# grossjohannes/AlignNet-3D

Hardware: AMD Instinct MI355X
Metric: point-cloud pairs/sec at N=1024 (inference, eval-mode forward) (higher is better)
Workload: dtype f32; 1 GPU; SynthCars widths inference, batch=256 pairs/GPU, N=1024, fp32 (BASELINE.json configs[1]); pairs_per_gpu=256, num_points=1024, parallelism=batch-split x1 (no collective)

## Files before the change

### alignnet-3d_amd/csrc/alignnet_api.hip

```cpp
#include "engine.h"
#include "kernels_infer.h"
#include "kernels_dgcnn.h"
#include "kernels_infer_split.h"
#include "kernels_dgcnn_split.h"

#include <algorithm>
#include <cmath>
#include <cstdio>
#include <cstring>
#include <random>

using namespace alignnet;

static thread_local std::string g_create_err;

#define HIP_TRY(h, expr)                                                                         \
  do {                                                                                           \
    hipError_t e_ = (expr);                                                                      \
    if (e_ != hipSuccess) {                                                                      \
      (h)->err = std::string(#expr) + ": " + hipGetErrorString(e_);                              \
      return 1;                                                                                  \
    }                                                                                            \
  } while (0)

// ... 343 lines not shown
    const size_t o_xform = tot; tot += al(B2 * 12);
    const size_t o_cm = tot; tot += al(B2 * 3);
    const size_t o_s1c = tot; tot += al(B2 * 3);
    const size_t o_s2c = tot; tot += al(B2 * 3);
    const size_t o_theta = tot; tot += al(B2);
    const size_t o_cls = tot; tot += al(B2);
    const size_t o_p1 = tot; tot += al(B2 * C1);
    const size_t o_p2 = tot; tot += al(B2 * C2);
    const size_t o_emb = tot; tot += al(B2 * CE);
    const size_t o_hs = tot; tot += al(B2 * H);
    const size_t o_ha = tot; tot += al(B2 * H);
    const size_t o_hb = tot; tot += al(B2 * H);
    const size_t o_o1 = tot; tot += al(B2 * 3);
    const size_t o_o2 = tot; tot += al(B2 * (3 + nb2));
    const size_t o_o3 = tot; tot += al((size_t)B * (3 + nb2));
    size_t o_out[8];
    const int widths[8] = {3, nb2, 3, 3, 3, 3, nb2, nb2};
    for (int i = 0; i < 8; ++i) { o_out[i] = tot; tot += al((size_t)B * widths[i]); }
    if (!(o_hs >= o_p1 && o_hs + al(B2 * H) <= o_ha)) return fail(h, "workspace carve: hid_s must lie inside the range the centroid kernel clears ([pool1, hid_a))");
    HIP_TRY(h, hipMalloc(&w.d_all, tot * sizeof(float)));
    float* base = w.d_all;
    w.xform = base + o_xform; w.center_mean = base + o_cm; w.s1c = base + o_s1c; w.s2c = base + o_s2c;
    w.theta = base + o_theta; w.cls = reinterpret_cast<int*>(base + o_cls);
    w.pool1 = base + o_p1; w.pool2 = base + o_p2; w.emb = base + o_emb;
    w.hid_a = base + o_ha; w.hid_b = base + o_hb; w.hid_s = base + o_hs;
    w.o1 = base + o_o1; w.o2 = base + o_o2; w.o3 = base + o_o3;
    for (int i = 0; i < 8; ++i) w.outs[i] = base + o_out[i];
    w.cap = B;
  }
  if (h->cfg.backbone == 1 && !w.d_nn) {
    HIP_TRY(h, hipMalloc(&w.d_nn, (size_t)2 * w.cap * N * 20 * sizeof(int)));
  }
  if (need_inputs && !w.d_pcs[0]) {
    for (int t = 0; t < 2; ++t) HIP_TRY(h, hipMalloc(&w.d_pcs[t], (size_t)w.cap * N * 3 * sizeof(float)));
  }
  return 0;
}

static int infer_tile_pts(const alignnet_handle* h, int B)
{
  if (h->ab & AB_INFER_TILE64) return 64;
  if (h->infer_tile_opt) return h->infer_tile_opt;
  const long tiles128 = (long)2 * B * ((h->cfg.num_points + 127) / 128);
  return tiles128 <= 128 ? 64 : 128;
}

static size_t backbone_lds_bytes(const alignnet_handle* h, const Stack& st, int ld[2], int B)
{
  const int kTilePts = infer_tile_pts(h, B);
  int w[2] = {8, 8};
  for (int i = 0; i < st.n - 1; ++i) w[i & 1] = std::max(w[i & 1], (h->layers[st.first + i].cout + 7) & ~7);
  ld[0] = w[0] + 4; ld[1] = w[1] + 4;
  return ((size_t)kTilePts * 4 + (size_t)kTilePts * (ld[0] + ld[1])) * sizeof(float);
}

static int run_backbone(alignnet_handle* h, const Stack& st, const float* p1, const float* p2, int B, float* pooled,
                        long tower_stride, long row_stride, size_t pooled_floats)
{
  BackboneArgs a;
  a.pcs[0] = p1; a.pcs[1] = p2; a.xform = h->ws.xform; a.pooled = pooled;
  a.tower_stride = tower_stride; a.row_stride = row_stride;
  a.B = B; a.N = h->cfg.num_points; a.nlayers = st.n;
  const size_t lds = backbone_lds_bytes(h, st, a.ld, B);
  if (lds > 160 * 1024) return fail(h, "backbone hidden widths need more than 160 KiB of LDS per 128-point tile");
  for (int i = 0; i < st.n; ++i) {
    const Layer& L = h->layers[st.first + i];
    a.L[i].w = L.first_conv ? h->d_params + h->params[L.p_w].offset : h->d_wp + L.off_wp;
    a.L[i].scale = h->d_scale + L.off_ss;
    a.L[i].shift = h->d_shift + L.off_ss;
    a.L[i].cin = L.cin; a.L[i].cout = L.cout;
  }
  (void)pooled_floats;
#ifdef ALIGNNET_KSTAMP
  static long long* d_stamps = nullptr;
  if (!d_stamps) { hipMalloc(&d_stamps, 4 * 64 * sizeof(long long)); }
  hipMemsetAsync(d_stamps, 0, 4 * 64 * sizeof(long long), h->stream);
  a.stamps = d_stamps;
#endif
  static PerDeviceOnce attr_set;
  if (attr_set.need(h->cfg.device)) {
    HIP_TRY(h, hipFuncSetAttribute(reinterpret_cast<const void*>(pointnet_fused<128>), hipFuncAttributeMaxDynamicSharedMemorySize, 160 * 1024));
    HIP_TRY(h, hipFuncSetAttribute(reinterpret_cast<const void*>(pointnet_fused<128, 68, 132>), hipFuncAttributeMaxDynamicSharedMemorySize, 160 * 1024));
    HIP_TRY(h, hipFuncSetAttribute(reinterpret_cast<const void*>(pointnet_fused<128, 68, 132, 16>), hipFuncAttributeMaxDynamicSharedMemorySize, 160 * 1024));
    HIP_TRY(h, hipFuncSetAttribute(reinterpret_cast<const void*>(pointnet_fused<64>), hipFuncAttributeMaxDynamicSharedMemorySize, 160 * 1024));
    HIP_TRY(h, hipFuncSetAttribute(reinterpret_cast<const void*>(pointnet_fused<64, 68, 132, 16>), hipFuncAttributeMaxDynamicSharedMemorySize, 160 * 1024));
    attr_set.mark(h->cfg.device);
  }
  const int TP = infer_tile_pts(h, B);
  const int ntiles = (a.N + TP - 1) / TP;
  int per = ntiles;
  while (per > 1 && (long)2 * B * ((ntiles + per - 1) / per) < 512) per = (per + 1) / 2;
  if (h->ab_tiles_per_wg > 0) per = std::min(ntiles, h->ab_tiles_per_wg);
  a.tiles_per_wg = per;
  const dim3 grid((ntiles + per - 1) / per, 2 * B);
  {
  ProfScope prof_scope(h, PK_BACKBONE, true);
  const int sc1 = h->layers[st.first].cout, sc2 = st.n == 3 ? h->layers[st.first + 1].cout : 0;
  if (h->infer_split && st.n == 3 && sc1 <= 16 * kSplitKB1 && sc2 <= 16 * kSplitKB2) {
    SplitArgs sa;
    sa.pcs[0] = p1; sa.pcs[1] = p2; sa.xform = a.xform; sa.pooled = pooled; sa.tower_stride = tower_stride; sa.row_stride = row_stride;
    sa.B = B; sa.N = a.N; sa.C1 = sc1; sa.C2 = sc2; sa.C3 = h->layers[st.first + 2].cout;
    sa.w1 = a.L[0].w; sa.w2s = h->d_wps + h->off_wps[st.first + 1]; sa.w3s = h->d_wps + h->off_wps[st.first + 2];
    sa.dbg = h->ablate_dbg & 0xff;
    if (h->ablate_dbg >> 8) sa.prio_mask = (h->ablate_dbg >> 8) & 0xff;
    sa.sc1 = a.L[0].scale; sa.sh1 = a.L[0].shift; sa.sc2 = a.L[1].scale; sa.sh2 = a.L[1].shift; sa.sc3 = a.L[2].scale; sa.sh3 = a.L[2].shift;
    const int ld1s = ((sc1 + 15) & ~15) + 8, ld2s = ((sc2 + 15) & ~15) + 8;
    const size_t slds = (size_t)kSplitTP * 4 * sizeof(float) + (size_t)2 * kSplitTP * (ld1s + ld2s) * sizeof(unsigned short);
    static PerDeviceOnce sattr;
    if (sattr.need(h->cfg.device)) { HIP_TRY(h, hipFuncSetAttribute(reinterpret_cast<const void*>(pointnet_split<>), hipFuncAttributeMaxDynamicSharedMemorySize, 160 * 1024)); sattr.mark(h->cfg.device); }
    if (sc1 == 64 && sc2 == 128 && sa.C3 % 64 == 0 && sa.C3 >= 256 && split_persist_lds(sa.C3).total_bytes <= 160 * 1024 && !(h->ab & (AB_NO_LD_CONST | AB_SPLIT_TILEWISE))) {
      static PerDeviceOnce pattr;
      static int cus[64];
      if (pattr.need(h->cfg.device)) {
        HIP_TRY(h, hipFuncSetAttribute(reinterpret_cast<const void*>(pointnet_split_persist<4>), hipFuncAttributeMaxDynamicSharedMemorySize, 160 * 1024));
        HIP_TRY(h, hipFuncSetAttribute(reinterpret_cast<const void*>(pointnet_split_persist<2>), hipFuncAttributeMaxDynamicSharedMemorySize, 160 * 1024));
        int n = 0;
        HIP_TRY(h, hipDeviceGetAttribute(&n, hipDeviceAttributeMultiprocessorCount, h->cfg.device));
        cus[h->cfg.device & 63] = n > 0 ? n : 256;
        pattr.mark(h->cfg.device);
      }
      const long tiles = (long)2 * B * ((a.N + kSplitTP - 1) / kSplitTP);
      const int wgs = (int)std::min<long>(tiles, cus[h->cfg.device & 63]);
      {
#ifdef ALIGNNET_ABLATE
      if ((sa.dbg & 64) && sa.C3 == 1024) { sa.stamps = reinterpret_cast<long long*>(h->ws.hid_a); hipMemsetAsync(sa.stamps, 0, 8 * 16 * sizeof(long long), h->stream); }
#endif
      if (sa.C3 >= 512) { TIMED_LAUNCH(pointnet_split_persist<4>, dim3(wgs), dim3(kWaves * 64), (size_t)split_persist_lds(sa.C3).total_bytes, sa); }
      else { TIMED_LAUNCH(pointnet_split_persist<2>, dim3(wgs), dim3(kWaves * 64), (size_t)split_persist_lds(sa.C3).total_bytes, sa); }
      h->last_kernel = ALIGNNET_KERNEL_POINTNET_SPLIT_PERSIST;
#ifdef ALIGNNET_ABLATE
      if (sa.stamps) {
        long long hs[8 * 16];
        hipStreamSynchronize(h->stream);
        hipMemcpy(hs, sa.stamps, sizeof(hs), hipMemcpyDeviceToHost);
        for (int w = 0; w < 8; ++w) {
          std::fprintf(stderr, "psp wave %d: start +%lld |", w, hs[w * 16] - hs[0]);
          for (int i = 1; i < 7; ++i) std::fprintf(stderr, " %lld", hs[w * 16 + i] - hs[w * 16 + i - 1]);
          std::fprintf(stderr, "   (xs+barrier, lift, barrier, hidden, barrier, last layer)\n");
        }
      }
#endif
      }
    } else if (sc1 == 64 && sc2 == 128 && !(h->ab & AB_NO_LD_CONST)) {
      static PerDeviceOnce sattr;
      if (sattr.need(h->cfg.device)) { HIP_TRY(h, hipFuncSetAttribute(reinterpret_cast<const void*>(pointnet_split<64, 128>), hipFuncAttributeMaxDynamicSharedMemorySize, 160 * 1024)); sattr.mark(h->cfg.device); }
      TIMED_LAUNCH((pointnet_split<64, 128>), dim3((a.N + kSplitTP - 1) / kSplitTP, 2 * B), dim3(kWaves * 64), slds, sa);
      h->last_kernel = ALIGNNET_KERNEL_POINTNET_SPLIT_64_128;
    } else {
      TIMED_LAUNCH(pointnet_split<>, dim3((a.N + kSplitTP - 1) / kSplitTP, 2 * B), dim3(kWaves * 64), slds, sa);
      h->last_kernel = ALIGNNET_KERNEL_POINTNET_SPLIT;
    }
  } else if (TP == 64 && !(h->ab & AB_INFER_TILE64) && a.ld[0] == 68 && a.ld[1] == 132 && st.n == 3 && h->layers[st.first + 2].cin == 128 && !(h->ab & AB_NO_LD_CONST)) {
    TIMED_LAUNCH((pointnet_fused<64, 68, 132, 16>), grid, dim3(kWaves * 64), lds, a);
    h->last_kernel = ALIGNNET_KERNEL_POINTNET_FUSED_64_128_K16_TP64;
  } else if (TP == 64) { TIMED_LAUNCH(pointnet_fused<64>, grid, dim3(kWaves * 64), lds, a); h->last_kernel = ALIGNNET_KERNEL_POINTNET_FUSED_TP64; }
  else if (a.ld[0] == 68 && a.ld[1] == 132 && st.n == 3 && h->layers[st.first + 2].cin == 128 && !(h->ab & AB_NO_LD_CONST)) {
    TIMED_LAUNCH((pointnet_fused<128, 68, 132, 16>), grid, dim3(kWaves * 64), lds, a);
    h->last_kernel = ALIGNNET_KERNEL_POINTNET_FUSED_64_128_K16;
  } else if (a.ld[0] == 68 && a.ld[1] == 132 && !(h->ab & AB_NO_LD_CONST)) {
    TIMED_LAUNCH((pointnet_fused<128, 68, 132>), grid, dim3(kWaves * 64), lds, a);
    h->last_kernel = ALIGNNET_KERNEL_POINTNET_FUSED_64_128;
  } else { TIMED_LAUNCH(pointnet_fused<128>, grid, dim3(kWaves * 64), lds, a); h->last_kernel = ALIGNNET_KERNEL_POINTNET_FUSED; }
  }
  HIP_TRY(h, hipGetLastError());
#ifdef ALIGNNET_KSTAMP
  if (st.first == h->emb_conv.first && true) {
    long long hs[4 * 64];
    hipStreamSynchronize(h->stream);
    hipMemcpy(hs, d_stamps, sizeof(hs), hipMemcpyDeviceToHost);
    for (int q = 0; q < 4; ++q) {
      std::fprintf(stderr, "wave %d ct %d:", (q >> 1) * 4, (q & 1) * 8 + (q >> 1) * 4);
      for (int i = 1; i < 64 && hs[q * 64 + i]; ++i) std::fprintf(stderr, " %lld", hs[q * 64 + i] - hs[q * 64 + i - 1]);
      std::fprintf(stderr, "  | first %lld\n", hs[q * 64] - hs[0]);
    }
  }
#endif
  return 0;
}

static int run_backbone_dgcnn(alignnet_handle* h, const Stack& st, const float* p1, const float* p2, int B, float* pooled,
                              long tower_stride, long row_stride, size_t pooled_floats)
{
  DgcnnArgs a;
  a.stamps = nullptr;
  a.pcs[0] = p1; a.pcs[1] = p2; a.xform = h->ws.xform; a.nn = h->ws.d_nn; a.pooled = pooled;
  a.tower_stride = tower_stride; a.row_stride = row_stride;
  a.B = B; a.N = h->cfg.num_points; a.k = 20; a.nlayers = st.n;
  int wmax[2] = {8, 8};
  for (int i = 0; i < st.n - 1; ++i) wmax[i & 1] = std::max(wmax[i & 1], (h->layers[st.first + i].cout + 7) & ~7);
  a.ld[0] = wmax[0] + 4; a.ld[1] = wmax[1] + 4;
  const bool dg_std = a.ld[0] == 68 && a.ld[1] == 132 && st.n == 3 && !(h->ab & AB_NO_LD_CONST);
  const size_t lds = dg_std ? ((size_t)kDgTile * 9 + (size_t)kDgTile * 68 + 4 * 8 * 64 * 4) * sizeof(float)
                            : ((size_t)kDgTile * 16 + (size_t)kDgTile * (2 * a.ld[0] + a.ld[1])) * sizeof(float);
  if (lds > 160 * 1024) return fail(h, "dgcnn hidden widths need more than 160 KiB of LDS per 64-point tile");
  if (h->layers[st.first + st.n - 2].cout > 256) return fail(h, "dgcnn: last edge-conv width limited to 256 channels");
  for (int i = 0; i < st.n; ++i) {
    const Layer& L = h->layers[st.first + i];
    a.L[i].w = L.first_conv ? h->d_params + h->params[L.p_w].offset : h->d_wp + L.off_wp;
    a.L[i].scale = h->d_scale + L.off_ss;
    a.L[i].shift = h->d_shift + L.off_ss;
    a.L[i].cin = L.cin; a.L[i].cout = L.cout;
  }
  (void)pooled_floats;
  static PerDeviceOnce attr_set;
  if (attr_set.need(h->cfg.device)) {
    HIP_TRY(h, hipFuncSetAttribute(reinterpret_cast<const void*>(dgcnn_fused<>), hipFuncAttributeMaxDynamicSharedMemorySize, 160 * 1024));
    attr_set.mark(h->cfg.device);
  }
  const dim3 grid((a.N + kDgTile - 1) / kDgTile, 2 * B);
  {
  ProfScope prof_scope(h, PK_BACKBONE, true);
  {
    const int dca = h->layers[st.first].cout, dcb = st.n == 3 ? h->layers[st.first + 1].cout : 0;
    if (h->infer_split && st.n == 3 && dca <= 16 * kSplitKB1 && dcb <= 128) {
      DgcnnSplitArgs sa;
      sa.pcs[0] = p1; sa.pcs[1] = p2; sa.xform = a.xform; sa.nn = a.nn; sa.pooled = pooled; sa.tower_stride = tower_stride; sa.row_stride = row_stride;
      sa.B = B; sa.N = a.N; sa.k = a.k; sa.Ca = dca; sa.Cb = dcb; sa.C3 = h->layers[st.first + 2].cout;
      sa.w1 = a.L[0].w; sa.w2s = h->d_wps + h->off_wps[st.first + 1]; sa.w3s = h->d_wps + h->off_wps[st.first + 2];
      sa.sc1 = a.L[0].scale; sa.sh1 = a.L[0].shift; sa.sc2 = a.L[1].scale; sa.sh2 = a.L[1].shift; sa.sc3 = a.L[2].scale; sa.sh3 = a.L[2].shift;
      sa.dbg = h->ablate_dbg;
      const int dlda = ((dca + 15) & ~15) + 8, dldb = ((dcb + 15) & ~15) + 8;
      if (a.k > 3 * kWaves) return fail(h, "dgcnn split kernel: k limited to 24 neighbours");
      const size_t dlds = (size_t)2 * kDgTile * 8 * sizeof(float) + ((size_t)4 * kDgTile * dlda + (size_t)2 * kDgTile * dldb) * sizeof(unsigned short);
      static PerDeviceOnce dsattr;
      if (dsattr.need(h->cfg.device)) { HIP_TRY(h, hipFuncSetAttribute(reinterpret_cast<const void*>(dgcnn_split<>), hipFuncAttributeMaxDynamicSharedMemorySize, 160 * 1024)); dsattr.mark(h->cfg.device); }
      if (dca == 64 && dcb == 128 && !(h->ab & AB_NO_LD_CONST)) {
        static PerDeviceOnce dsattr2;
        if (dsattr2.need(h->cfg.device)) { HIP_TRY(h, hipFuncSetAttribute(reinterpret_cast<const void*>(dgcnn_split<64, 128>), hipFuncAttributeMaxDynamicSharedMemorySize, 160 * 1024)); dsattr2.mark(h->cfg.device); }
        TIMED_LAUNCH((dgcnn_split<64, 128>), grid, dim3(kWaves * 64), dlds, sa);
        h->last_kernel = ALIGNNET_KERNEL_DGCNN_SPLIT_64_128;
      } else {
        TIMED_LAUNCH(dgcnn_split<>, grid, dim3(kWaves * 64), dlds, sa);
        h->last_kernel = ALIGNNET_KERNEL_DGCNN_SPLIT;
      }
    } else {
      const int dbg = h->ablate_dbg;
      a.stamps = (dbg & 64) ? reinterpret_cast<long long*>(h->ws.hid_a) : nullptr;
      if (a.ld[0] == 68 && a.ld[1] == 132 && st.n == 3 && !(h->ab & AB_NO_LD_CONST)) {
        static PerDeviceOnce sattr;
        if (sattr.need(h->cfg.device)) { HIP_TRY(h, hipFuncSetAttribute(reinterpret_cast<const void*>(dgcnn_fused<68, 132>), hipFuncAttributeMaxDynamicSharedMemorySize, 160 * 1024)); sattr.mark(h->cfg.device); }
// ... 455 lines not shown
```

### alignnet-3d_amd/csrc/engine.h

```cpp
#pragma once
#include <hip/hip_runtime.h>
#include <hip/hip_ext.h>
#include <stdint.h>
#include <string>
#include <vector>
#include <map>
#include <atomic>

#include "../../include/alignnet_hip.h"

namespace alignnet {

struct ParamInfo {
  std::string name;
  int rows, cols;
  bool trainable;
  size_t offset;
  size_t count() const { return (size_t)rows * cols; }
};

struct Layer {
  std::string name;
  int cin, cout;
  bool bn, siamese, conv, first_conv;
  int fan_in, fan_out;
  int p_w, p_b;
  int p_bn[2][4];
  size_t off_wp;
  size_t off_ss;
};

struct Stack { int first, n; };

enum ProfKernel { PK_BACKBONE = 0, PK_KNN, PK_TRAIN_PHASE2, PK_TRAIN_PHASE3, PK_TRAIN_GRAM, PK_TRAIN_B2, PK_TRAIN_B1, PK_DG_FWD, PK_DG_BWD_EDGE,
                  PK_ALLREDUCE, PK_OPTIMIZER, PK_SCENE_WINDOW, PK_SCENE_CAST, PK_SCENE_COMPACT, PK_ICP_GRID_BUILD, PK_ICP_GRID, PK_SCENE_BIN, PK_ICP_PLANE_NORMALS, PK_ICP_PLANE, PK_SCENE_BAND, PK_TRACKLET_TEST, PK_TRACKLET_COMPACT, PK_COUNT };
static const char* const kProfKernelNames[PK_COUNT] = {"backbone", "knn", "train_fwd_phase2", "train_fwd_phase3", "train_gram_h2", "train_bwd_b2",
                                                       "train_bwd_b1", "dg_train_fwd", "dg_train_bwd_edge", "allreduce", "optimizer", "scene_window", "scene_cast", "scene_compact", "icp_grid_build", "icp_grid", "scene_bin", "icp_plane_normals", "icp_plane", "scene_band", "tracklet_test", "tracklet_compact"};

constexpr int kTrackletChunk = 1024;
constexpr int kTrackletJobsPerPass = 32;

struct Workspace {
  int cap = 0;
  float* d_pcs[2] = {nullptr, nullptr};
  int* d_nn = nullptr;
  float* d_all = nullptr;
  float *xform, *center_mean, *s1c, *s2c, *theta;
  int* cls;
  float *pool1, *pool2, *emb;
  float *hid_a, *hid_b;
  float* hid_s;
  bool hid_s_zeroed = false;
  float *o1, *o2, *o3;
  float* outs[8];
};

}

namespace alignnet {
struct DatasetTables { const float* pts[2]; const long long* off; long long n; const long long* h_off; const float* labels; };
struct SampleSource { const float* pts[2]; const long long* off; const float* labels; const int* rows; const long long* streams; };
struct IcpDeviceIo {
  const double* init; double* out; double* fitness; double* rmse; int* iters;
  long long* ws_off;
  std::vector<long long>* h_ws_off;
};
}
enum AbBit : unsigned {
  AB_NO_LD_CONST = 1u << 0,
  AB_INFER_TILE64 = 1u << 1,
  AB_PHASE2_LEGACY = 1u << 2,
  AB_B1_LEGACY = 1u << 3,
  AB_B1_FP32 = 1u << 4,
  AB_P3BF16_GENERIC = 1u << 5,
  AB_P3_NOGRAM = 1u << 6,
  AB_NO_DEFER = 1u << 7,
  AB_DG_SPARSE = 1u << 8,
  AB_NO_GLUE_FOLD = 1u << 9,
  AB_FC_DIRECT = 1u << 11,
  AB_FC_NO_SPLITK = 1u << 12,
  AB_SPLIT_TILEWISE = 1u << 13,
  AB_GEMM_JOBS_KSPLIT = 1u << 10,
};
static const struct { const char* key; unsigned bit; } kAbKeys[] = {
  {"ab_no_ld_const", AB_NO_LD_CONST}, {"ab_infer_tile64", AB_INFER_TILE64}, {"ab_phase2_legacy", AB_PHASE2_LEGACY}, {"ab_b1_legacy", AB_B1_LEGACY},
  {"ab_b1_fp32", AB_B1_FP32}, {"ab_p3_bf16_generic", AB_P3BF16_GENERIC}, {"ab_p3_nogram", AB_P3_NOGRAM}, {"ab_no_defer", AB_NO_DEFER},
  {"ab_dg_sparse", AB_DG_SPARSE}, {"ab_no_glue_fold", AB_NO_GLUE_FOLD}, {"ab_gemm_jobs_ksplit", AB_GEMM_JOBS_KSPLIT}, {"ab_fc_direct", AB_FC_DIRECT}, {"ab_fc_no_splitk", AB_FC_NO_SPLITK}, {"ab_split_tilewise", AB_SPLIT_TILEWISE}};
struct alignnet_handle;
bool alignnet_dataset_tables(alignnet_handle* h, alignnet::DatasetTables* out);
int alignnet_dataset_install(alignnet_handle* h, const float* points1, const float* points2, bool device_points, const int64_t* offsets, const float* labels,
                             int64_t n_examples, const char* fn);
int alignnet_dataset_sample_launch(alignnet_handle* h, const alignnet::SampleSource& s, int B, int cap, uint64_t seed, float* out0, float* out1,
                                   float* lab, alignnet_labels* lab_ptrs);
int alignnet_icp_run_device(alignnet_handle* h, const float* const pts[2], const long long* off, const int* rows, const long long* n2, long long stage_n2,
                            int B, const alignnet::IcpDeviceIo& io, double radius, double normal_radius, int its, bool full, bool plane);
size_t alignnet_eval_loss_work_floats(int B);
int alignnet_eval_loss_launch(alignnet_handle* h, const alignnet_labels* d_labels, int B, float* d_work);
void alignnet_register_free(alignnet_handle* h);
int alignnet_drain_profile(alignnet_handle* h);
int alignnet_train_set_option(alignnet_handle* h, const std::string& key, int64_t value);
int alignnet_train_get_option(alignnet_handle* h, const std::string& key, int64_t* value);

struct alignnet_handle {
  alignnet_config cfg;
  std::vector<alignnet::Layer> layers;
  alignnet::Stack s1_conv, s1_fc, s2_conv, s2_fc, emb_conv, rem_fc;
  std::vector<alignnet::ParamInfo> params;
  std::map<std::string, int> by_name;
  size_t n_trainable = 0, n_total = 0;
  float* d_params = nullptr;
  float* d_wp = nullptr;
  float* d_scale = nullptr;
  float* d_shift = nullptr;
  size_t n_wp = 0, n_ss = 0;
  bool infer_split = false;
  unsigned short* d_wps = nullptr;
  std::vector<size_t> off_wps;
  bool train_bf16 = false;
  bool fused_tail = true;
  bool train_ws_stale = false;
  bool folded = false;
  alignnet::Workspace ws;
  hipStream_t stream = nullptr;
  int64_t step = 0;
  uint64_t dropout_stream = 0;
  float adam_b1p = 1.f, adam_b2p = 1.f;
  int64_t adam_power_t = 0;
  int last_B = 0;
  int last_kernel = 0;
  int last_train_B = 0;
  int last_train_kernel = 0;
  bool prof = false;
  hipEvent_t ev[2] = {nullptr, nullptr};
  double prof_backbone_ms = 0, prof_total_ms = 0;
  int64_t prof_backbone_launches = 0;
  struct ProfEv { int id; hipEvent_t a, b; };
  std::vector<ProfEv> prof_pending;
  std::vector<std::pair<hipEvent_t, hipEvent_t>> prof_pool;
  double prof_ms[alignnet::PK_COUNT] = {0};
  int64_t prof_launches[alignnet::PK_COUNT] = {0};
  void* train_ws = nullptr;
  void* dataset_ws = nullptr;
  void* globalreg_ws = nullptr;
  size_t globalreg_ws_bytes = 0;
  int icp_search = 0;
  void* register_ws = nullptr;
  void* icp_grid_ws = nullptr;
  size_t icp_grid_ws_bytes = 0, icp_grid_ws_used = 0;
  size_t icp_plane_ws_budget = 0;
  int icp_plane_chunks = 0;
  int scene_cast = 0;
  int scene_rows = 0;
  int scene_binned_clouds = 0;
  long long scene_bin_entries = 0;
  void* scene_ws = nullptr;
  void* tracklet_ws = nullptr;
  void* pipe = nullptr;
  uint64_t dropout_seed_base() const { return (cfg.seed + dropout_stream * 0xD1B54A32D192ED03ull) * 0x9E3779B97F4A7C15ull + (uint64_t)step * 16; }
  void* comm = nullptr;
  void* comm_grad = nullptr;
  int comm_world = 1, comm_rank = 0;
  hipStream_t comm_stream = nullptr;
  hipEvent_t comm_ev[4] = {nullptr, nullptr, nullptr, nullptr};
  bool comm_overlap = true;
  hipStream_t side_stream = nullptr;
  hipEvent_t side_ev[4] = {nullptr, nullptr, nullptr, nullptr};
  int dw_side = 0;
  unsigned ab = 0;
  int infer_tile_opt = 0;
  int dg_parts_opt = 0;
// ... 45 lines not shown
```

### alignnet-3d_amd/csrc/kernels_infer.h

```cpp
#pragma once
#include <hip/hip_runtime.h>
#include <stdint.h>

namespace alignnet {

typedef __attribute__((ext_vector_type(16))) float f32x16;
typedef __attribute__((ext_vector_type(4))) float f32x4;

constexpr int kTilePts = 128;
constexpr int kWaves = 8;
constexpr int kMaxConv = 6;
constexpr float kBnEps = 1e-3f;

#ifndef ALIGNNET_NO_SETPRIO
#define ALIGNNET_SETPRIO 1
#endif

[[maybe_unused]] static __global__ void pack_weights_kernel(const float* __restrict__ W, int K, int C, float* __restrict__ Wp)
{
  const int KG = (K + 7) >> 3, CT = (C + 31) >> 5;
  const size_t total = (size_t)CT * KG * 256;
  for (size_t idx = blockIdx.x * (size_t)blockDim.x + threadIdx.x; idx < total; idx += (size_t)gridDim.x * blockDim.x) {
    const int s = idx & 3, lane = (idx >> 2) & 63;
    const size_t t = idx >> 8;
// ... 181 lines not shown
    b2 = wload_issue(wp + min(kg + 2, last) * 64);
    lds_rows<MR>(arow, lda, min(kg + 1, last), a1);
    wload_wait2(b0);
    KSTAMP();
    mfma_kgroup<MR>(a0, b0, acc);
    KSTAMP();
    b0 = wload_issue(wp + min(kg + 3, last) * 64);
    lds_rows<MR>(arow, lda, min(kg + 2, last), a0);
    wload_wait2(b1);
    if (kg + 1 < KG) mfma_kgroup<MR>(a1, b1, acc);
    b1 = wload_issue(wp + min(kg + 4, last) * 64);
    lds_rows<MR>(arow, lda, min(kg + 3, last), a1);
    wload_wait2(b2);
    if (kg + 2 < KG) mfma_kgroup<MR>(a0, b2, acc);
#pragma unroll
    for (int m = 0; m < MR; ++m) a0[m] = a1[m];
  }
  KSTAMP();
  wload_drain(b0, b1, b2);
  KSTAMP();
}

template <int MR, bool CLEAR = true>
__device__ __forceinline__ void mfma_rows_deep(const float* __restrict__ A, int lda, const f32x4* __restrict__ Wp, int KG, int lane,
                                               f32x16 (&acc)[MR])
{
  if (CLEAR) {
#pragma unroll
    for (int m = 0; m < MR; ++m)
#pragma unroll
      for (int r = 0; r < 16; ++r) acc[m][r] = 0.f;
  }
  const float* arow = A + (lane & 31) * lda + (lane >> 5) * 4;
  const f32x4* wp = Wp + lane;
  const int last = KG - 1;
  f32x4 b0 = wp[0], b1 = wp[min(1, last) * 64], b2 = wp[min(2, last) * 64];
  asm volatile("" ::: "memory");
  f32x4 av[MR];
  for (int kg = 0; kg < KG; kg += 3) {
    lds_rows<MR>(arow, lda, kg, av);
    mfma_kgroup<MR>(av, b0, acc);
    b0 = wp[min(kg + 3, last) * 64];
    asm volatile("" ::: "memory");
    if (kg + 1 < KG) { lds_rows<MR>(arow, lda, kg + 1, av); mfma_kgroup<MR>(av, b1, acc); }
    b1 = wp[min(kg + 4, last) * 64];
    asm volatile("" ::: "memory");
    if (kg + 2 < KG) { lds_rows<MR>(arow, lda, kg + 2, av); mfma_kgroup<MR>(av, b2, acc); }
    b2 = wp[min(kg + 5, last) * 64];
    asm volatile("" ::: "memory");
  }
}

template <int MR, int KGC = 0>
__device__ __forceinline__ void hidden_item(const float* __restrict__ in, int ldi, float* __restrict__ out, int ldo,
                                            const ConvLayerDev& L, int tower, int ct, int rg, int lane)
{
  const int KG = KGC ? KGC : (L.cin + 7) >> 3;
  f32x16 acc[MR];
  mfma_rows<MR>(in + rg * MR * 32 * ldi, ldi, reinterpret_cast<const f32x4*>(L.w) + (size_t)ct * KG * 64, KG, lane, acc);
  const int col = ct * 32 + (lane & 31);
  const bool live = col < L.cout;
  const float sc = live ? L.scale[tower * L.cout + col] : 0.f;
  const float sh = live ? L.shift[tower * L.cout + col] : 0.f;
  if (col < ldo - 4) {
#pragma unroll
    for (int m = 0; m < MR; ++m)
#pragma unroll
      for (int r = 0; r < 16; ++r) {
        const int row = (rg * MR + m) * 32 + (r & 3) + 8 * (r >> 2) + 4 * (lane >> 5);
        out[row * ldo + col] = fmaxf(fmaf(acc[m][r], sc, sh), 0.f);
      }
  }
}

template <int MR, int TP>
__device__ __forceinline__ void hidden_layer(const float* in, int ldi, float* out, int ldo, const ConvLayerDev& L,
                                             int tower, int wave, int lane)
{
  constexpr int RG = (TP / 32) / MR;
  const int CT = (L.cout + 31) >> 5;
  for (int item = wave; item < CT * RG; item += kWaves) hidden_item<MR>(in, ldi, out, ldo, L, tower, item / RG, item % RG, lane);
}

template <int TP, int LD0 = 0, int LD1 = 0, int KGL = 0>
__global__ __launch_bounds__(kWaves * 64, 2) void pointnet_fused(const BackboneArgs a)
{
  const int lds_ld[2] = {LD0 ? LD0 : a.ld[0], LD1 ? LD1 : a.ld[1]};
  extern __shared__ __attribute__((aligned(16))) float smem[];
  const int tid = threadIdx.x, lane = tid & 63;
  const int wave = __builtin_amdgcn_readfirstlane(tid >> 6);
  const int cloud = blockIdx.y;
  const int tower = cloud >= a.B, b = cloud - tower * a.B;
  float* xs = smem;
  const int boff[2] = {TP * 4, TP * 4 + TP * lds_ld[0]};
  constexpr int kPoolRegs = 4;
  float pool[kPoolRegs] = {0.f, 0.f, 0.f, 0.f};
  const int ntiles_all = (a.N + TP - 1) / TP;
  const int tile_lo = blockIdx.x * a.tiles_per_wg, tile_hi = min(ntiles_all, tile_lo + a.tiles_per_wg);
  float nx = 0.f, ny = 0.f, nz = 0.f;
  auto request_xyz = [&](int t) {
    if (tid < TP) {
      const int n = min(t * TP + tid, a.N - 1);
      const float* p = a.pcs[tower] + ((size_t)b * a.N + n) * 3;
      nx = p[0]; ny = p[1]; nz = p[2];
    }
  };
  request_xyz(tile_lo);
  float l0w[2][5];
#pragma unroll
  for (int g = 0; g < 2; ++g) {
    const ConvLayerDev& L0 = a.L[0];
    const int c = (tid & 31) + 32 * g;
    const bool live = c < L0.cout;
    l0w[g][0] = live ? L0.w[c] : 0.f; l0w[g][1] = live ? L0.w[L0.cout + c] : 0.f; l0w[g][2] = live ? L0.w[2 * L0.cout + c] : 0.f;
    l0w[g][3] = live ? L0.scale[tower * L0.cout + c] : 0.f; l0w[g][4] = live ? L0.shift[tower * L0.cout + c] : 0.f;
  }
  for (int tile = tile_lo; tile < tile_hi; ++tile) {
  if (tile != tile_lo) __syncthreads();

  if (tid < TP) {
    const float* xf = a.xform + (size_t)cloud * 12;
    const float x = nx - xf[0], y = ny - xf[1], z = nz - xf[2];
    xs[tid * 4 + 0] = x * xf[3] + y * xf[6] + z * xf[9];
    xs[tid * 4 + 1] = x * xf[4] + y * xf[7] + z * xf[10];
    xs[tid * 4 + 2] = x * xf[5] + y * xf[8] + z * xf[11];
  }
  if (tile + 1 < tile_hi) request_xyz(tile + 1);
  __syncthreads();

  {
    const ConvLayerDev& L = a.L[0];
    float* out = smem + boff[0];
    const int ldo = lds_ld[0], c0 = tid & 31, r0 = tid >> 5;
    for (int c = c0; c < ldo - 4; c += 32) {
      const bool live = c < L.cout;
      const int g = (c - c0) >> 5;
      float w0, w1, w2, sc, sh;
      if (g < 2) { w0 = g ? l0w[1][0] : l0w[0][0]; w1 = g ? l0w[1][1] : l0w[0][1]; w2 = g ? l0w[1][2] : l0w[0][2];
                   sc = g ? l0w[1][3] : l0w[0][3]; sh = g ? l0w[1][4] : l0w[0][4]; }
      else { w0 = live ? L.w[c] : 0.f; w1 = live ? L.w[L.cout + c] : 0.f; w2 = live ? L.w[2 * L.cout + c] : 0.f;
             sc = live ? L.scale[tower * L.cout + c] : 0.f; sh = live ? L.shift[tower * L.cout + c] : 0.f; }
#pragma unroll
      for (int rr = 0; rr < TP / 16; ++rr) {
        const int row = rr * 16 + r0;
        const f32x4 p = *reinterpret_cast<const f32x4*>(xs + row * 4);
        const float acc = fmaf(p[2], w2, fmaf(p[1], w1, p[0] * w0));
        out[row * ldo + c] = fmaxf(fmaf(acc, sc, sh), 0.f);
      }
    }
  }
  __syncthreads();

  if constexpr (KGL != 0 && LD0 != 0 && LD1 != 0) {
    constexpr int CTH = (LD1 - 4) / 32, RGH = (TP / 32) / 2;
    for (int item = wave; item < CTH * RGH; item += kWaves)
      hidden_item<2, (LD0 - 4) / 8>(smem + boff[0], LD0, smem + boff[1], LD1, a.L[1], tower, item / RGH, item % RGH, lane);
    __syncthreads();
  } else
  for (int l = 1; l < a.nlayers - 1; ++l) {
    const ConvLayerDev& L = a.L[l];
    const int CT = (L.cout + 31) >> 5;
    const float* in = smem + (((l - 1) & 1) ? boff[1] : boff[0]);
    float* out = smem + ((l & 1) ? boff[1] : boff[0]);
    const int ldi = lds_ld[(l - 1) & 1], ldo = lds_ld[l & 1];
    constexpr int MT = TP / 32;
    if (CT >= kWaves) hidden_layer<MT, TP>(in, ldi, out, ldo, L, tower, wave, lane);
    else if (CT * 2 >= kWaves || MT < 4) hidden_layer<(MT >= 2 ? 2 : 1), TP>(in, ldi, out, ldo, L, tower, wave, lane);
    else hidden_layer<1, TP>(in, ldi, out, ldo, L, tower, wave, lane);
    __syncthreads();
  }

  {
    const int l = a.nlayers - 1;
    const ConvLayerDev& L = a.L[l];
    const float* in = smem + (((l - 1) & 1) ? boff[1] : boff[0]);
    const int ldi = lds_ld[(l - 1) & 1];
    const int KG = (LD1 && KGL) ? KGL : (L.cin + 7) >> 3, CT = (L.cout + 31) >> 5;
    float* dst = a.pooled + tower * a.tower_stride + b * a.row_stride;
    for (int ct = wave; ct < CT; ct += kWaves) {
      f32x16 acc[TP / 32];
      const int col = ct * 32 + (lane & 31);
      const bool live = col < L.cout;
      const float sc = live ? L.scale[tower * L.cout + col] : 0.f;
      const float sh = live ? L.shift[tower * L.cout + col] : 0.f;
      asm volatile("" ::: "memory");
#ifdef ALIGNNET_KSTAMP
      long long* kst = (a.stamps && blockIdx.x == 0 && blockIdx.y == 1 && tile == tile_lo + 2 && lane == 0 && (wave == 0 || wave == 4) && ct < 16)
                           ? a.stamps + ((wave >> 2) * 2 + (ct >> 3)) * 64 : nullptr;
      if (kst) *kst++ = (long long)__builtin_readcyclecounter();
      mfma_rows<TP / 32>(in, ldi, reinterpret_cast<const f32x4*>(L.w) + (size_t)ct * KG * 64, KG, lane, acc, kst);
#else
      mfma_rows<TP / 32>(in, ldi, reinterpret_cast<const f32x4*>(L.w) + (size_t)ct * KG * 64, KG, lane, acc);
#endif
      float mx = 0.f;
#pragma unroll
      for (int m = 0; m < TP / 32; ++m)
#pragma unroll
        for (int r = 0; r < 16; ++r) mx = fmaxf(mx, fmaf(acc[m][r], sc, sh));
      const int q = (ct - wave) / kWaves;
      if (q < kPoolRegs) {
#pragma unroll
        for (int u = 0; u < kPoolRegs; ++u)
          if (u == q) pool[u] = fmaxf(pool[u], mx);
      } else {
        mx = fmaxf(mx, __shfl_xor(mx, 32));
        if (lane < 32 && live) atomicMax(reinterpret_cast<int*>(dst + col), __float_as_int(mx));
      }
    }
  }
  }
  {
    const ConvLayerDev& L = a.L[a.nlayers - 1];
    const int CT = (L.cout + 31) >> 5;
    float* dst = a.pooled + tower * a.tower_stride + b * a.row_stride;
#pragma unroll
    for (int u = 0; u < kPoolRegs; ++u) {
      const int ct = wave + u * kWaves, col = ct * 32 + (lane & 31);
      if (ct < CT) {
        const float mx = fmaxf(pool[u], __shfl_xor(pool[u], 32));
        if (lane < 32 && col < L.cout) atomicMax(reinterpret_cast<int*>(dst + col), __float_as_int(mx));
      }
    }
  }
}

struct FcArgs {
  const float* in; long ldin;
  const float* wp; const float* scale; const float* shift;
  float* out; long ldout;
  int M, K, Nout, relu, rows_per_set;
  int finish = 0; int B = 0, nb = 0;
  const float* addend = nullptr;
  float* s1c = nullptr; float* xform = nullptr;
  float* out_a = nullptr; float* out_b = nullptr;
  int ksplit = 1;
  const float* in_scale = nullptr; const float* in_shift = nullptr;
};

constexpr int kFcLd = 68;
template <int NW, bool STAGE = false>
static __global__ __launch_bounds__(NW * 64) void fc_mfma(const FcArgs a)
{
  __shared__ float red[NW - 1][16][64];
  __shared__ __attribute__((aligned(16))) float stageA[STAGE ? NW : 1][STAGE ? 32 * kFcLd : 4];
  const int lane = threadIdx.x & 63, wave = __builtin_amdgcn_readfirstlane(threadIdx.x >> 6);
  const int ct = blockIdx.x, mt = blockIdx.y;
  const int KG = a.K >> 3;
  const int row_in = min(mt * 32 + (lane & 31), a.M - 1);
  const float* arow = a.in + (size_t)row_in * a.ldin + (lane >> 5) * 4;
  const f32x4* wp = reinterpret_cast<const f32x4*>(a.wp) + (size_t)ct * KG * 64 + lane;
  f32x16 acc;
#pragma unroll
  for (int r = 0; r < 16; ++r) acc[r] = 0.f;
  const int KGz = KG / a.ksplit, kz0 = (int)blockIdx.z * KGz;
  const int per = (KGz + NW - 1) / NW, k0 = kz0 + wave * per, k1 = min(kz0 + KGz, k0 + per);
  float add0[16], add1[16];
#pragma unroll
  for (int r = 0; r < 16; ++r) { add0[r] = 0.f; add1[r] = 0.f; }
  if (a.finish && ct == 0) {
    const int col = lane & 31;
#pragma unroll
    for (int r = 0; r < 16; ++r) {
      const int row = min(mt * 32 + (r & 3) + 8 * (r >> 2) + 4 * (lane >> 5), a.M - 1);
      add0[r] = col < 3 ? a.addend[row * 3 + col] : 0.f;
      add1[r] = (a.finish == 3 && col < 3) ? a.addend[(a.B + row) * 3 + col] : 0.f;
    }
  }
  const int ecol = min(ct * 32 + (lane & 31), a.Nout - 1);
  const float esc0 = a.scale[ecol], esh0 = a.shift[ecol], esc1 = a.scale[a.Nout + ecol], esh1 = a.shift[a.Nout + ecol];
  constexpr int U = 8;
  for (int kg = k0; kg < k1; kg += U) {
    f32x4 av[U], bv[U];
    if (STAGE) {
      float* st = stageA[wave];
#pragma unroll
      for (int u = 0; u < U; ++u) {
        const int q = u * 64 + lane, r = q >> 4, c16 = q & 15;
        const int kk = min(kg + (c16 >> 1), k1 - 1);
        const int row_g = min(mt * 32 + r, a.M - 1);
        av[u] = *reinterpret_cast<const f32x4*>(a.in + (size_t)row_g * a.ldin + kk * 8 + (c16 & 1) * 4);
        bv[u] = wp[(size_t)min(kg + u, k1 - 1) * 64];
      }
      if (a.in_scale) {
#pragma unroll
        for (int u = 0; u < U; ++u) {
          const int c16 = (u * 64 + lane) & 15, kk = min(kg + (c16 >> 1), k1 - 1);
          const f32x4 sc = *reinterpret_cast<const f32x4*>(a.in_scale + kk * 8 + (c16 & 1) * 4);
          const f32x4 sh = *reinterpret_cast<const f32x4*>(a.in_shift + kk * 8 + (c16 & 1) * 4);
#pragma unroll
          for (int e = 0; e < 4; ++e) av[u][e] = fmaxf(fmaf(av[u][e], sc[e], sh[e]), 0.f);
        }
      }
#pragma unroll
      for (int u = 0; u < U; ++u) {
        const int q = u * 64 + lane, r = q >> 4, c16 = q & 15;
        *reinterpret_cast<f32x4*>(st + r * kFcLd + c16 * 4) = av[u];
      }
      __builtin_amdgcn_wave_barrier();
#pragma unroll
      for (int u = 0; u < U; ++u) av[u] = *reinterpret_cast<const f32x4*>(st + (lane & 31) * kFcLd + u * 8 + (lane >> 5) * 4);
      __builtin_amdgcn_wave_barrier();
    } else {
#pragma unroll
    for (int u = 0; u < U; ++u) {
      const int kk = min(kg + u, k1 - 1);
      av[u] = *reinterpret_cast<const f32x4*>(arow + kk * 8);
      bv[u] = wp[(size_t)kk * 64];
    }
// ... 140 lines not shown
```

Before: 122,000 pairs/s.

## Row-serial last PointNet layer with register-resident weights and overlapped epilogue

Restructures the last conv layer of the fused PointNet backbone for 128-point tiles with K depth 16. Each wave now keeps its column tile's weights in registers across tiles. It walks the four 32-row blocks serially, prefetching A rows three deep from LDS. While the next MFMA chain runs, it applies scale/shift and the max-pool to the previous accumulator, and reloads the next tile's weights inside the final chain. The goal is to cut repeated weight fetches and hide epilogue latency behind MFMA issue, at the cost of much higher VGPR pressure under launch bounds of 2 blocks. That pressure risks spills or lower occupancy. The old path stays reachable through a new ablation flag, even though that flag is confusingly named 'stream'.

```diff
diff --git a/alignnet-3d_amd/csrc/alignnet_api.hip b/alignnet-3d_amd/csrc/alignnet_api.hip
--- a/alignnet-3d_amd/csrc/alignnet_api.hip
+++ b/alignnet-3d_amd/csrc/alignnet_api.hip
@@ -449,6 +449,7 @@
     HIP_TRY(h, hipFuncSetAttribute(reinterpret_cast<const void*>(pointnet_fused<128>), hipFuncAttributeMaxDynamicSharedMemorySize, 160 * 1024));
     HIP_TRY(h, hipFuncSetAttribute(reinterpret_cast<const void*>(pointnet_fused<128, 68, 132>), hipFuncAttributeMaxDynamicSharedMemorySize, 160 * 1024));
     HIP_TRY(h, hipFuncSetAttribute(reinterpret_cast<const void*>(pointnet_fused<128, 68, 132, 16>), hipFuncAttributeMaxDynamicSharedMemorySize, 160 * 1024));
+    HIP_TRY(h, hipFuncSetAttribute(reinterpret_cast<const void*>(pointnet_fused_stream<128, 68, 132, 16>), hipFuncAttributeMaxDynamicSharedMemorySize, 160 * 1024));
     HIP_TRY(h, hipFuncSetAttribute(reinterpret_cast<const void*>(pointnet_fused<64>), hipFuncAttributeMaxDynamicSharedMemorySize, 160 * 1024));
     HIP_TRY(h, hipFuncSetAttribute(reinterpret_cast<const void*>(pointnet_fused<64, 68, 132, 16>), hipFuncAttributeMaxDynamicSharedMemorySize, 160 * 1024));
     attr_set.mark(h->cfg.device);
@@ -522,7 +523,13 @@
     h->last_kernel = ALIGNNET_KERNEL_POINTNET_FUSED_64_128_K16_TP64;
   } else if (TP == 64) { TIMED_LAUNCH(pointnet_fused<64>, grid, dim3(kWaves * 64), lds, a); h->last_kernel = ALIGNNET_KERNEL_POINTNET_FUSED_TP64; }
   else if (a.ld[0] == 68 && a.ld[1] == 132 && st.n == 3 && h->layers[st.first + 2].cin == 128 && !(h->ab & AB_NO_LD_CONST)) {
-    TIMED_LAUNCH((pointnet_fused<128, 68, 132, 16>), grid, dim3(kWaves * 64), lds, a);
+#ifdef ALIGNNET_KSTAMP
+    const bool stream = true;
+#else
+    const bool stream = h->ab & AB_LAST_LAYER_STREAM;
+#endif
+    if (stream) { TIMED_LAUNCH((pointnet_fused_stream<128, 68, 132, 16>), grid, dim3(kWaves * 64), lds, a); }
+    else { TIMED_LAUNCH((pointnet_fused<128, 68, 132, 16>), grid, dim3(kWaves * 64), lds, a); }
     h->last_kernel = ALIGNNET_KERNEL_POINTNET_FUSED_64_128_K16;
   } else if (a.ld[0] == 68 && a.ld[1] == 132 && !(h->ab & AB_NO_LD_CONST)) {
     TIMED_LAUNCH((pointnet_fused<128, 68, 132>), grid, dim3(kWaves * 64), lds, a);
diff --git a/alignnet-3d_amd/csrc/engine.h b/alignnet-3d_amd/csrc/engine.h
--- a/alignnet-3d_amd/csrc/engine.h
+++ b/alignnet-3d_amd/csrc/engine.h
@@ -80,12 +80,14 @@
   AB_FC_DIRECT = 1u << 11,
   AB_FC_NO_SPLITK = 1u << 12,
   AB_SPLIT_TILEWISE = 1u << 13,
+  AB_LAST_LAYER_STREAM = 1u << 14,
   AB_GEMM_JOBS_KSPLIT = 1u << 10,
 };
 static const struct { const char* key; unsigned bit; } kAbKeys[] = {
   {"ab_no_ld_const", AB_NO_LD_CONST}, {"ab_infer_tile64", AB_INFER_TILE64}, {"ab_phase2_legacy", AB_PHASE2_LEGACY}, {"ab_b1_legacy", AB_B1_LEGACY},
   {"ab_b1_fp32", AB_B1_FP32}, {"ab_p3_bf16_generic", AB_P3BF16_GENERIC}, {"ab_p3_nogram", AB_P3_NOGRAM}, {"ab_no_defer", AB_NO_DEFER},
-  {"ab_dg_sparse", AB_DG_SPARSE}, {"ab_no_glue_fold", AB_NO_GLUE_FOLD}, {"ab_gemm_jobs_ksplit", AB_GEMM_JOBS_KSPLIT}, {"ab_fc_direct", AB_FC_DIRECT}, {"ab_fc_no_splitk", AB_FC_NO_SPLITK}, {"ab_split_tilewise", AB_SPLIT_TILEWISE}};
+  {"ab_dg_sparse", AB_DG_SPARSE}, {"ab_no_glue_fold", AB_NO_GLUE_FOLD}, {"ab_gemm_jobs_ksplit", AB_GEMM_JOBS_KSPLIT}, {"ab_fc_direct", AB_FC_DIRECT}, {"ab_fc_no_splitk", AB_FC_NO_SPLITK}, {"ab_split_tilewise", AB_SPLIT_TILEWISE},
+  {"ab_last_layer_stream", AB_LAST_LAYER_STREAM}};
 struct alignnet_handle;
 bool alignnet_dataset_tables(alignnet_handle* h, alignnet::DatasetTables* out);
 int alignnet_dataset_install(alignnet_handle* h, const float* points1, const float* points2, bool device_points, const int64_t* offsets, const float* labels,
diff --git a/alignnet-3d_amd/csrc/kernels_infer.h b/alignnet-3d_amd/csrc/kernels_infer.h
--- a/alignnet-3d_amd/csrc/kernels_infer.h
+++ b/alignnet-3d_amd/csrc/kernels_infer.h
@@ -287,9 +287,35 @@
   for (int item = wave; item < CT * RG; item += kWaves) hidden_item<MR>(in, ldi, out, ldo, L, tower, item / RG, item % RG, lane);
 }
 
-template <int TP, int LD0 = 0, int LD1 = 0, int KGL = 0>
-__global__ __launch_bounds__(kWaves * 64, 2) void pointnet_fused(const BackboneArgs a)
-{
+template <int KG, int M, bool RELOAD>
+__device__ __forceinline__ void rowserial_chain(const float* arow, int lda, f32x4 (&bw)[KG], const f32x4* __restrict__ wnext, f32x4 (&av)[3],
+                                                f32x16& acc, const f32x16& prev, float sc, float sh, float& mx)
+{
+  constexpr int MT = 4;
+  const f32x16 zero = {0.f, 0.f, 0.f, 0.f, 0.f, 0.f, 0.f, 0.f, 0.f, 0.f, 0.f, 0.f, 0.f, 0.f, 0.f, 0.f};
+#pragma unroll
+  for (int kg = 0; kg < KG; ++kg) {
+    const int t = M * KG + kg;
+    if (t + 2 < MT * KG) av[(t + 2) % 3] = *reinterpret_cast<const f32x4*>(arow + ((t + 2) / KG) * 32 * lda + ((t + 2) % KG) * 8);
+#pragma unroll
+    for (int s = 0; s < 4; ++s) {
+      if (kg == 0 && s == 0) acc = __builtin_amdgcn_mfma_f32_32x32x2f32(av[t % 3][s], bw[kg][s], zero, 0, 0, 0);
+      else acc = __builtin_amdgcn_mfma_f32_32x32x2f32(av[t % 3][s], bw[kg][s], acc, 0, 0, 0);
+    }
+    if (kg >= 1 && kg <= 4) {
+#pragma unroll
+      for (int r = 0; r < 4; ++r) mx = fmaxf(mx, fmaf(prev[(kg - 1) * 4 + r], sc, sh));
+    }
+    if (RELOAD) bw[kg] = wnext[kg * 64];
+    asm volatile("" ::: "memory");
+    __builtin_amdgcn_sched_barrier(0);
+  }
+}
+
+template <int TP, int LD0, int LD1, int KGL, bool ROWSER>
+__device__ __forceinline__ void pointnet_fused_body(const BackboneArgs& a)
+{
+  static_assert(!ROWSER || (TP == 128 && LD1 != 0 && KGL != 0), "row-serial last layer: 128-point tiles, compile-time depth");
   const int lds_ld[2] = {LD0 ? LD0 : a.ld[0], LD1 ? LD1 : a.ld[1]};
   extern __shared__ __attribute__((aligned(16))) float smem[];
   const int tid = threadIdx.x, lane = tid & 63;
@@ -320,6 +346,14 @@
     l0w[g][0] = live ? L0.w[c] : 0.f; l0w[g][1] = live ? L0.w[L0.cout + c] : 0.f; l0w[g][2] = live ? L0.w[2 * L0.cout + c] : 0.f;
     l0w[g][3] = live ? L0.scale[tower * L0.cout + c] : 0.f; l0w[g][4] = live ? L0.shift[tower * L0.cout + c] : 0.f;
   }
+  [[maybe_unused]] f32x4 bw[ROWSER ? KGL : 1];
+  if constexpr (ROWSER) {
+    if (wave * 32 < a.L[a.nlayers - 1].cout) {
+      const f32x4* wp = reinterpret_cast<const f32x4*>(a.L[a.nlayers - 1].w) + (size_t)wave * KGL * 64 + lane;
+#pragma unroll
+      for (int kg = 0; kg < KGL; ++kg) bw[kg] = wp[kg * 64];
+    }
+  }
   for (int tile = tile_lo; tile < tile_hi; ++tile) {
   if (tile != tile_lo) __syncthreads();
 
@@ -375,7 +409,54 @@
     __syncthreads();
   }
 
-  {
+  if constexpr (ROWSER) {
+    const ConvLayerDev& L = a.L[a.nlayers - 1];
+    const int CT = (L.cout + 31) >> 5;
+    const float* arow = smem + boff[1] + (lane & 31) * LD1 + (lane >> 5) * 4;
+    float* dst = a.pooled + tower * a.tower_stride + b * a.row_stride;
+    auto retire = [&](float m, int q, bool live, int col) {
+      if (q < kPoolRegs) {
+#pragma unroll
+        for (int u = 0; u < kPoolRegs; ++u)
+          if (u == q) pool[u] = fmaxf(pool[u], m);
+      } else {
+        m = fmaxf(m, __shfl_xor(m, 32));
+        if (lane < 32 && live) atomicMax(reinterpret_cast<int*>(dst + col), __float_as_int(m));
+      }
+    };
+    f32x16 acc0, acc1;
+#pragma unroll
+    for (int r = 0; r < 16; ++r) acc1[r] = 0.f;
+    float scp = 0.f, shp = 0.f, mx = 0.f;
+    int qp = 0, colp = 0;
+    bool livep = false;
+    for (int ct = wave; ct < CT; ct += kWaves) {
+      const int col = ct * 32 + (lane & 31);
+      const bool live = col < L.cout;
+      const float sc = live ? L.scale[tower * L.cout + col] : 0.f;
+      const float sh = live ? L.shift[tower * L.cout + col] : 0.f;
+      const int nct = ct + kWaves < CT ? ct + kWaves : wave;
+      const bool reload = nct != ct && (ct + kWaves < CT || tile + 1 < tile_hi);
+      const f32x4* wnext = reinterpret_cast<const f32x4*>(L.w) + (size_t)nct * KGL * 64 + lane;
+      f32x4 av[3];
+      av[0] = *reinterpret_cast<const f32x4*>(arow);
+      av[1] = *reinterpret_cast<const f32x4*>(arow + 8);
+      asm volatile("" ::: "memory");
+      rowserial_chain<KGL, 0, false>(arow, LD1, bw, wnext, av, acc0, acc1, scp, shp, mx);
+      retire(mx, qp, livep, colp);
+      mx = 0.f;
+      rowserial_chain<KGL, 1, false>(arow, LD1, bw, wnext, av, acc1, acc0, sc, sh, mx);
+      rowserial_chain<KGL, 2, false>(arow, LD1, bw, wnext, av, acc0, acc1, sc, sh, mx);
+      if (reload) rowserial_chain<KGL, 3, true>(arow, LD1, bw, wnext, av, acc1, acc0, sc, sh, mx);
+      else rowserial_chain<KGL, 3, false>(arow, LD1, bw, wnext, av, acc1, acc0, sc, sh, mx);
+      scp = sc; shp = sh; qp = (ct - wave) / kWaves; colp = col; livep = live;
+    }
+    if (wave < CT) {
+#pragma unroll
+      for (int r = 0; r < 16; ++r) mx = fmaxf(mx, fmaf(acc1[r], scp, shp));
+      retire(mx, qp, livep, colp);
+    }
+  } else {
     const int l = a.nlayers - 1;
     const ConvLayerDev& L = a.L[l];
     const float* in = smem + (((l - 1) & 1) ? boff[1] : boff[0]);
@@ -429,6 +510,17 @@
   }
 }
 
+template <int TP, int LD0 = 0, int LD1 = 0, int KGL = 0>
+__global__ __launch_bounds__(kWaves * 64, 2) void pointnet_fused(const BackboneArgs a)
+{
+  pointnet_fused_body<TP, LD0, LD1, KGL, TP == 128 && LD0 == 68 && LD1 == 132 && KGL == 16>(a);
+}
+template <int TP, int LD0, int LD1, int KGL>
+__global__ __launch_bounds__(kWaves * 64, 2) void pointnet_fused_stream(const BackboneArgs a)
+{
+  pointnet_fused_body<TP, LD0, LD1, KGL, false>(a);
+}
+
 struct FcArgs {
   const float* in; long ldin;
   const float* wp; const float* scale; const float* shift;
```

Result: faster. 126,300 pairs/s (median of 6 runs) (+3.5%).
